# huangnengCSU/NanoSNP

Measured on NVIDIA B200. Metric: candidate sites/sec (s1+s2), higher is better.
Workload: dtype int32 counts, fp64 AF gate, fp16 hi/lo split x3 tensor-core model (fp32 accumulate)

## Files before the change

### nanosnp_b200/csrc/model_tc.cu

```cuda
#include <cuda_fp16.h>
#include <stdlib.h>
#include "model_common.cuh"
#include "tc_ptx.cuh"

namespace nsnp {
namespace {

constexpr int kRows = 128;
constexpr float kLog2e = 1.4426950408889634f;

__device__ __forceinline__ uint4 scale_hi(const uint4& hi) {
    const __half2 k = __float2half2_rn(1.0f / kTcLoScale);
    auto m = [&](uint32_t x) { __half2 t = *reinterpret_cast<__half2*>(&x); return h2_bits(__hmul2(t, k)); };
    return make_uint4(m(hi.x), m(hi.y), m(hi.z), m(hi.w));
}

template <int LAYER> struct TcCfg;
template <> struct TcCfg<0> { static constexpr int K = kTcK0, IN = kTcIn0, STEPS = 33; };
template <> struct TcCfg<1> { static constexpr int K = kTcK1, IN = kTcIn1, STEPS = 17; };

template <int LAYER, int CG> struct TcSmem {
    static constexpr int K = TcCfg<LAYER>::K;
    static constexpr int RB = 256 / CG;
    static constexpr size_t b_bytes = (size_t)K * RB * 2;
// ... 204 lines not shown
        }

        uint32_t vb[2][16];
        const uint32_t tacc = tmem_base + acc_cols + ((uint32_t)(quad * 32) << 16) + (uint32_t)(sub * UB) * 32u;
        tmem_ld16_nowait(tacc, vb[0]);
        tmem_wait_ld();
        float hv[8];
#pragma unroll
        for (int hb = 0; hb < 2 * UB; ++hb) {
            const int jl = hb >> 1, uh = hb & 1, jb = sub * UB + jl;
            if (hb + 1 < 2 * UB) tmem_ld16_nowait(tacc + (hb + 1) * 16, vb[(hb + 1) & 1]);
#pragma unroll
            for (int u = 0; u < 4; ++u) {
                const uint32_t* v = vb[hb & 1];
                const float* bq = sBias + jb * 32 + uh * 16 + u;
                const float bi_ = LAYER == 1 ? bq[0] : 0.f, bf_ = LAYER == 1 ? bq[4] : 0.f, bg_ = LAYER == 1 ? bq[8] : 0.f, bo_ = LAYER == 1 ? bq[12] : 0.f;
                const float xi_ = fminf(__uint_as_float(v[u]) + bi_, 36.f), xf_ = fminf(__uint_as_float(v[4 + u]) + bf_, 36.f);
                const float xg_ = fminf(__uint_as_float(v[8 + u]) + bg_, 36.f), xo_ = __uint_as_float(v[12 + u]) + bo_;
                const float ei = ex2_approx(xi_), ef = ex2_approx(xf_), eg = ex2_approx(xg_), eo = ex2_approx(xo_);
                const float pi = 1.f + ei, pf = 1.f + ef, pg = 1.f + eg;
                const float pig = pi * pg;
                const float num = fmaf(c[jl][uh * 4 + u], pig, fmaf(eg, 2.f * kLog2e, -2.f * kLog2e) * pf);
                const float cn = num * rcp_approx(pf * pig);
                c[jl][uh * 4 + u] = cn;
                const float ec = ex2_approx(cn);
                hv[uh * 4 + u] = (1.f - ec) * rcp_approx((1.f + eo) * (1.f + ec));
            }
            if (hb + 1 < 2 * UB) tmem_wait_ld();
            if (uh == 1) {
                const HiLo8 s = split8(hv);
                reinterpret_cast<uint4*>(sAhi + (IN / 8 + jb) * LBO_A)[row] = s.hi;
                reinterpret_cast<uint4*>(sAlo + (IN / 8 + jb) * LBO_A)[row] = s.lo;
                if (live) {
                    if (LAYER == 0) {
                        __half* o = h0_out + ((((size_t)blockIdx.x * kT + t) * 2) * 16 + (dir * 8 + jb)) * (kRows * 8) + row * 8;
                        *reinterpret_cast<uint4*>(o) = s.hi;
                        *reinterpret_cast<uint4*>(o + 16 * kRows * 8) = s.lo;
                    } else if (step == C::STEPS - 1) {
                        float4* o = reinterpret_cast<float4*>(h16 + site * 128 + dir * kH + jb * 8);
                        o[0] = make_float4(hv[0], hv[1], hv[2], hv[3]); o[1] = make_float4(hv[4], hv[5], hv[6], hv[7]);
                    }
                }
            }
        }
        if (more) store_x();
    }

    tc_fence_before();
    if (CG == 2) cluster_sync_all(); else __syncthreads();
    if (warp == 0) tmem_dealloc<CG>(tmem_base, kTmemCols);
}


__device__ __forceinline__ void mbar_arrive(uint64_t* bar) {
    asm volatile("mbarrier.arrive.shared::cta.b64 _, [%0];" ::"r"(smem_u32(bar)) : "memory");
}

constexpr int kP2GroupThreads = 256, kP2Threads = 2 * kP2GroupThreads;
struct P2Smem {
    static constexpr size_t b_bytes = (size_t)kTcK0 * 128 * 2;
    static constexpr size_t a_bytes = (size_t)kTcK0 * kRows * 2;
    static constexpr size_t sc_bytes = (size_t)kTcIn0 * kRows * 2;
    static constexpr size_t a_stride = 2 * a_bytes + sc_bytes;
    static constexpr size_t off_bhi = 0, off_blo = b_bytes, off_a = 2 * b_bytes, off_bar = off_a + 2 * a_stride, total = off_bar + 128;
};

__global__ void __launch_bounds__(kP2Threads, 1)
lstm0_pair2_kernel(const unsigned char* __restrict__ blob, const int32_t* __restrict__ xi, const float* __restrict__ xf,
                   __half* __restrict__ h0_out, int64_t n, const int32_t* __restrict__ pos, int64_t pos_bias, int npass)
{
    using S = P2Smem;
    constexpr int K = kTcK0, IN = kTcIn0, KB = K / 16, RB = 128, UB = 4;
    constexpr uint32_t LBO_A = kRows * 16, LBO_B = RB * 16, SBO = 128;
    extern __shared__ __align__(1024) unsigned char smem[];
    const int grp = (int)threadIdx.x / kP2GroupThreads;
    const int tid = (int)threadIdx.x - grp * kP2GroupThreads, lane = tid & 31, warp = tid >> 5;
    unsigned char* sBhi = smem + S::off_bhi; unsigned char* sBlo = smem + S::off_blo;
    unsigned char* sAhi = smem + S::off_a + grp * S::a_stride; unsigned char* sAlo = sAhi + S::a_bytes; unsigned char* sAsc = sAlo + S::a_bytes;
    uint64_t* bars = reinterpret_cast<uint64_t*>(smem + S::off_bar);
    uint64_t* barH = bars + grp;
    uint64_t* barReady = bars + 2 + grp;
    uint64_t* barTurn = bars + 4;
    uint32_t* tmem_slot = reinterpret_cast<uint32_t*>(smem + S::off_bar + 64);

    const int quad = warp & 3, sub = warp >> 2;
    const int row = quad * 32 + lane;
    const uint32_t cta_rank = cluster_ctarank();
    const int cluster_id = (int)(blockIdx.x >> 1);
    const int dir = cluster_id & 1;
    const int quad_stride = (int)(gridDim.x >> 2);
    const int n_quads = (int)((n + 4 * kRows - 1) / (4 * kRows));
    const int q0 = cluster_id >> 1;
    const int my_quads = q0 < n_quads ? (n_quads - q0 + quad_stride - 1) / quad_stride : 0;
    const int total_g = my_quads * kT;
    auto tile_of = [&](int qi) -> int64_t { return (int64_t)(q0 + qi * quad_stride) * 4 + (int64_t)cta_rank * 2 + grp; };

    if (threadIdx.x == 0) {
        mbar_init(bars + 0, 1); mbar_init(bars + 1, 1); mbar_init(bars + 2, 16); mbar_init(bars + 3, 16);
        mbar_init(bars + 4, 1); mbar_init(bars + 5, 1);
        fence_mbar_init();
    }
    if (threadIdx.x < 32) tmem_alloc<2>(tmem_slot, 512);
    {
        const uint4* ghi = reinterpret_cast<const uint4*>(blob + tc_off(0, dir, 0));
        const uint4* glo = reinterpret_cast<const uint4*>(blob + tc_off(0, dir, 1));
        uint4* dhi = reinterpret_cast<uint4*>(sBhi); uint4* dlo = reinterpret_cast<uint4*>(sBlo);
        for (int i = (int)threadIdx.x; i < (K / 8) * RB; i += kP2Threads) {
            const int ch = i / RB, r = i - ch * RB;
            const int g = ch * 256 + (int)cta_rank * RB + r;
            dhi[i] = __ldg(ghi + g); dlo[i] = __ldg(glo + g);
        }
        uint4* a = reinterpret_cast<uint4*>(sAhi);
        for (int i = tid; i < (int)(S::a_stride / 16); i += kP2GroupThreads) a[i] = make_uint4(0, 0, 0, 0);
    }
    __syncthreads();

    float c[UB][8];
#pragma unroll
    for (int j = 0; j < UB; ++j)
#pragma unroll
        for (int u = 0; u < 8; ++u) c[j][u] = 0.f;

    int2 xraw[8];
    int64_t win0 = 0;
    auto load_x = [&](int gstep) {
        const int qi = gstep / kT, st = gstep - qi * kT;
        const int t = dir == 0 ? st : (kT - 1 - st);
        int64_t site = tile_of(qi) * kRows + row;
        if (site >= n) site = n - 1;
        if (pos && st == 0) win0 = (int64_t)__ldg(pos + site) - pos_bias;
        const int2* g = pos ? reinterpret_cast<const int2*>(xi + (win0 + t) * kF)
                            : reinterpret_cast<const int2*>(xi ? (const void*)(xi + (site * kT + t) * kF) : (const void*)(xf + (site * kT + t) * kF));
        if (sub == 0) {
#pragma unroll
            for (int j = 0; j < 8; ++j) xraw[j] = ldg_nc_volatile(g + j);
        } else {
            xraw[0] = ldg_nc_volatile(g + 8);
        }
    };
    auto xval = [&](int j) -> float {
        const int2 p = xraw[j >> 1];
        const int b = (j & 1) ? p.y : p.x;
        return xi ? (float)b : __int_as_float(b);
    };
    auto store_x = [&]() {
        if (sub == 0) {
#pragma unroll
            for (int ch = 0; ch < 2; ++ch) {
                float v[8];
#pragma unroll
                for (int j = 0; j < 8; ++j) v[j] = xval(ch * 8 + j);
                const HiLo8 sp = split8(v);
                reinterpret_cast<uint4*>(sAhi + ch * LBO_A)[row] = sp.hi;
                reinterpret_cast<uint4*>(sAlo + ch * LBO_A)[row] = sp.lo;
                reinterpret_cast<uint4*>(sAsc + ch * LBO_A)[row] = scale_hi(sp.hi);
            }
        } else {
            const float v[8] = {xval(0), xval(1), 1.0f, 0.f, 0.f, 0.f, 0.f, 0.f};
            const HiLo8 sp = split8(v);
            reinterpret_cast<uint4*>(sAhi + 2 * LBO_A)[row] = sp.hi;
            reinterpret_cast<uint4*>(sAlo + 2 * LBO_A)[row] = sp.lo;
            reinterpret_cast<uint4*>(sAsc + 2 * LBO_A)[row] = scale_hi(sp.hi);
        }
    };
    auto report_ready = [&]() {
        fence_async_smem();
        tc_fence_before();
        __syncwarp();
        if (lane == 0) mbar_arrive_remote_relaxed(barReady, 0);
    };
    if (total_g > 0) { load_x(0); store_x(); }
    tc_fence_before();
    cluster_sync_all();
    tc_fence_after();
    if (total_g > 0) report_ready();

    const uint32_t tmem_base = *tmem_slot + (uint32_t)grp * 256u;
    const uint32_t a_hi = smem_u32(sAhi), a_lo = smem_u32(sAlo), a_sc = smem_u32(sAsc), b_hi = smem_u32(sBhi), b_lo = smem_u32(sBlo);
    constexpr uint32_t idesc = make_idesc(256, 256);
    const bool issuer = cta_rank == 0 && tid == 0;
    uint32_t phaseH = 0, phaseR = 0, phaseT = 0;
    if (cta_rank == 0 && threadIdx.x == 0) mbar_arrive(barTurn + 0);

    int step = 0, qi = 0;
    for (int g = 0; g < total_g; ++g) {
        const int t = dir == 0 ? step : (kT - 1 - step);
        const bool more = g + 1 < total_g;
        const int64_t tile_idx = tile_of(qi);
        const bool live = tile_idx * kRows + row < n;
        if (step == 0) {
#pragma unroll
            for (int j = 0; j < UB; ++j)
#pragma unroll
                for (int u = 0; u < 8; ++u) c[j][u] = 0.f;
        }
        if (issuer) {
            mbar_wait_cluster(barReady, phaseR);
            mbar_wait(barTurn + grp, phaseT);
            tc_fence_after();
#pragma unroll 1
            for (int pass = 0; pass < npass; ++pass) {
#pragma unroll 1
                for (int kb = 0; kb < (step == 0 ? IN / 16 : KB); ++kb) {
                    uint32_t aa = pass == 2 ? a_lo : a_hi;
                    if (pass == 1 && kb < IN / 16) aa = a_sc;
                    const uint32_t bb = pass == 1 ? b_lo : b_hi;
                    umma_f16<2>(tmem_base, make_desc(aa + kb * 2 * LBO_A, LBO_A, SBO), make_desc(bb + kb * 2 * LBO_B, LBO_B, SBO), idesc,
                                (pass | kb) ? 1u : 0u);
                }
            }
            umma_commit<2>(barH);
            mbar_arrive(barTurn + (grp ^ 1));
        }
        phaseR ^= 1; phaseT ^= 1;
        if (more) load_x(g + 1);
        mbar_wait(barH, phaseH);
        phaseH ^= 1;
        tc_fence_after();

        uint32_t vb[2][16];
        const uint32_t tacc = tmem_base + ((uint32_t)(quad * 32) << 16) + (uint32_t)(sub * UB) * 32u;
        tmem_ld16_nowait(tacc, vb[0]);
        tmem_wait_ld();
        float hv[8];
#pragma unroll
        for (int hb = 0; hb < 2 * UB; ++hb) {
            const int jl = hb >> 1, uh = hb & 1, jb = sub * UB + jl;
            if (hb + 1 < 2 * UB) tmem_ld16_nowait(tacc + (hb + 1) * 16, vb[(hb + 1) & 1]);
#pragma unroll
            for (int u = 0; u < 4; ++u) {
                const uint32_t* v = vb[hb & 1];
                const float xi_ = fminf(__uint_as_float(v[u]), 36.f), xf_ = fminf(__uint_as_float(v[4 + u]), 36.f);
                const float xg_ = fminf(__uint_as_float(v[8 + u]), 36.f), xo_ = __uint_as_float(v[12 + u]);
                const float ei = ex2_approx(xi_), ef = ex2_approx(xf_), eg = ex2_approx(xg_), eo = ex2_approx(xo_);
                const float pi = 1.f + ei, pf = 1.f + ef, pg = 1.f + eg;
                const float pig = pi * pg;
                const float num = fmaf(c[jl][uh * 4 + u], pig, fmaf(eg, 2.f * kLog2e, -2.f * kLog2e) * pf);
                const float cn = num * rcp_approx(pf * pig);
                c[jl][uh * 4 + u] = cn;
                const float ec = ex2_approx(cn);
                hv[uh * 4 + u] = (1.f - ec) * rcp_approx((1.f + eo) * (1.f + ec));
            }
            if (hb + 1 < 2 * UB) tmem_wait_ld();
            if (uh == 1) {
                const HiLo8 sp = split8(hv);
                reinterpret_cast<uint4*>(sAhi + (IN / 8 + jb) * LBO_A)[row] = sp.hi;
                if (npass == 3) reinterpret_cast<uint4*>(sAlo + (IN / 8 + jb) * LBO_A)[row] = sp.lo;
                if (live) {
                    __half* o = h0_out + ((((size_t)tile_idx * kT + t) * 2) * 16 + (dir * 8 + jb)) * (kRows * 8) + row * 8;
                    *reinterpret_cast<uint4*>(o) = sp.hi;
                    if (npass == 3) *reinterpret_cast<uint4*>(o + 16 * kRows * 8) = sp.lo;
                }
            }
        }
        if (more) { store_x(); report_ready(); }
        if (++step == kT) { step = 0; ++qi; }
    }

    tc_fence_before();
    cluster_sync_all();
    if (threadIdx.x < 32) tmem_dealloc<2>(*tmem_slot, 512);
}

struct P2Smem1 {
    static constexpr size_t b_bytes = (size_t)kTcK1 * 128 * 2;
    static constexpr size_t a_bytes = (size_t)kTcK1 * kRows * 2;
    static constexpr size_t off_b = 0, off_a = b_bytes, off_bias = off_a + 2 * a_bytes, off_bar = off_bias + 256 * sizeof(float), total = off_bar + 128;
};

__global__ void __launch_bounds__(kP2Threads, 1)
lstm1_pair2_kernel(const unsigned char* __restrict__ blob, const __half* __restrict__ h0_in, float* __restrict__ h16, int64_t n)
{
    using S = P2Smem1;
    constexpr int K = kTcK1, IN = kTcIn1, KB = K / 16, XB = IN / 16, RB = 128, UB = 4, kS = TcCfg<1>::STEPS;
    constexpr uint32_t LBO_A = kRows * 16, LBO_B = RB * 16, SBO = 128;
    constexpr uint32_t kPartBytes = 16u * kRows * 16u;
    extern __shared__ __align__(1024) unsigned char smem[];
    const int grp = (int)threadIdx.x / kP2GroupThreads;
    const int tid = (int)threadIdx.x - grp * kP2GroupThreads, lane = tid & 31, warp = tid >> 5;
    unsigned char* sB = smem + S::off_b;
    unsigned char* sA = smem + S::off_a + grp * S::a_bytes;
    float* sBias = reinterpret_cast<float*>(smem + S::off_bias);
    uint64_t* bars = reinterpret_cast<uint64_t*>(smem + S::off_bar);
    uint64_t* barH = bars + grp;
    uint64_t* barReady = bars + 2 + grp;
    uint64_t* barTurn = bars + 4;
    uint64_t* barIn = bars + 6 + grp;
    uint32_t* tmem_slot = reinterpret_cast<uint32_t*>(smem + S::off_bar + 64);

    const int quad = warp & 3, sub = warp >> 2;
    const int row = quad * 32 + lane;
    const uint32_t cta_rank = cluster_ctarank();
    const int cluster_id = (int)(blockIdx.x >> 1);
    const int dir = cluster_id & 1;
    const int quad_stride = (int)(gridDim.x >> 2);
    const int n_quads = (int)((n + 4 * kRows - 1) / (4 * kRows));
    const int64_t last_tile = (n + kRows - 1) / kRows - 1;
    const int q0 = cluster_id >> 1;
    const int my_quads = q0 < n_quads ? (n_quads - q0 + quad_stride - 1) / quad_stride : 0;
    const int total_g = my_quads * kS;
    auto tile_of = [&](int qi) -> int64_t { return (int64_t)(q0 + qi * quad_stride) * 4 + (int64_t)cta_rank * 2 + grp; };

    if (threadIdx.x == 0) {
        mbar_init(bars + 0, 1); mbar_init(bars + 1, 1); mbar_init(bars + 2, 16); mbar_init(bars + 3, 16);
        mbar_init(bars + 4, 1); mbar_init(bars + 5, 1); mbar_init(bars + 6, 1); mbar_init(bars + 7, 1);
        fence_mbar_init();
    }
    if (threadIdx.x < 32) tmem_alloc<2>(tmem_slot, 512);
    {
        const uint4* ghi = reinterpret_cast<const uint4*>(blob + tc_off(1, dir, 0));
        uint4* dhi = reinterpret_cast<uint4*>(sB);
        for (int i = (int)threadIdx.x; i < (K / 8) * RB; i += kP2Threads) {
            const int ch = i / RB, r = i - ch * RB;
            dhi[i] = __ldg(ghi + ch * 256 + (int)cta_rank * RB + r);
        }
        const float* gb = reinterpret_cast<const float*>(blob + kOffTcBias1) + dir * 256;
        for (int i = (int)threadIdx.x; i < 256; i += kP2Threads) sBias[i] = __ldg(gb + i);
    }
    __syncthreads();

    float c[UB][8];
#pragma unroll
    for (int j = 0; j < UB; ++j)
#pragma unroll
        for (int u = 0; u < 8; ++u) c[j][u] = 0.f;

    auto stage_in = [&](int gstep) {
        const int qi = gstep / kS, st = gstep - qi * kS;
        const int t = dir == 0 ? st : (kT - 1 - st);
        const int64_t tile = min(tile_of(qi), last_tile);
        mbar_expect_tx(barIn, kPartBytes);
        bulk_g2s(sA, h0_in + ((size_t)tile * kT + t) * (size_t)kPartBytes, kPartBytes, barIn);
    };
    auto report_ready = [&]() {
        fence_async_smem();
        tc_fence_before();
        __syncwarp();
        if (lane == 0) mbar_arrive_remote_relaxed(barReady, 0);
// ... 8 lines not shown
        report_ready();
    }

    const uint32_t tmem_base = *tmem_slot + (uint32_t)grp * 256u;
    const uint32_t a_hi = smem_u32(sA), b_hi = smem_u32(sB);
    constexpr uint32_t idesc = make_idesc(256, 256);
    const bool issuer = cta_rank == 0 && tid == 0;
    uint32_t phaseH = 0, phaseR = 0, phaseT = 0;
    if (cta_rank == 0 && threadIdx.x == 0) mbar_arrive(barTurn + 0);

    int step = 0, qi = 0;
    for (int g = 0; g < total_g; ++g) {
        const bool more = g + 1 < total_g;
        const int64_t site = tile_of(qi) * kRows + row;
        const bool live = site < n;
        if (step == 0) {
#pragma unroll
            for (int j = 0; j < UB; ++j)
#pragma unroll
                for (int u = 0; u < 8; ++u) c[j][u] = 0.f;
        }
        if (issuer) {
            mbar_wait_cluster(barReady, phaseR);
            mbar_wait(barTurn + grp, phaseT);
            tc_fence_after();
#pragma unroll 1
            for (int kb = 0; kb < (step == 0 ? XB : KB); ++kb)
                umma_f16<2>(tmem_base, make_desc(a_hi + kb * 2 * LBO_A, LBO_A, SBO), make_desc(b_hi + kb * 2 * LBO_B, LBO_B, SBO), idesc, kb ? 1u : 0u);
            umma_commit<2>(barH);
            mbar_arrive(barTurn + (grp ^ 1));
        }
        phaseR ^= 1; phaseT ^= 1;
        mbar_wait(barH, phaseH);
        phaseH ^= 1;
        tc_fence_after();
        if (more && tid == 0) stage_in(g + 1);

        uint32_t vb[2][16];
        const uint32_t tacc = tmem_base + ((uint32_t)(quad * 32) << 16) + (uint32_t)(sub * UB) * 32u;
        tmem_ld16_nowait(tacc, vb[0]);
        tmem_wait_ld();
        float hv[8];
#pragma unroll
        for (int hb = 0; hb < 2 * UB; ++hb) {
            const int jl = hb >> 1, uh = hb & 1, jb = sub * UB + jl;
            if (hb + 1 < 2 * UB) tmem_ld16_nowait(tacc + (hb + 1) * 16, vb[(hb + 1) & 1]);
#pragma unroll
            for (int u = 0; u < 4; ++u) {
                const uint32_t* v = vb[hb & 1];
                const float* bq = sBias + jb * 32 + uh * 16 + u;
                const float xi_ = fminf(__uint_as_float(v[u]) + bq[0], 36.f), xf_ = fminf(__uint_as_float(v[4 + u]) + bq[4], 36.f);
                const float xg_ = fminf(__uint_as_float(v[8 + u]) + bq[8], 36.f), xo_ = __uint_as_float(v[12 + u]) + bq[12];
                const float ei = ex2_approx(xi_), ef = ex2_approx(xf_), eg = ex2_approx(xg_), eo = ex2_approx(xo_);
                const float pi = 1.f + ei, pf = 1.f + ef, pg = 1.f + eg;
                const float pig = pi * pg;
                const float num = fmaf(c[jl][uh * 4 + u], pig, fmaf(eg, 2.f * kLog2e, -2.f * kLog2e) * pf);
                const float cn = num * rcp_approx(pf * pig);
                c[jl][uh * 4 + u] = cn;
                const float ec = ex2_approx(cn);
                hv[uh * 4 + u] = (1.f - ec) * rcp_approx((1.f + eo) * (1.f + ec));
            }
            if (hb + 1 < 2 * UB) tmem_wait_ld();
            if (uh == 1) {
                const HiLo8 sp = split8(hv);
                reinterpret_cast<uint4*>(sA + (IN / 8 + jb) * LBO_A)[row] = sp.hi;
                if (live && step == kS - 1) {
                    float4* o = reinterpret_cast<float4*>(h16 + site * 128 + dir * kH + jb * 8);
                    o[0] = make_float4(hv[0], hv[1], hv[2], hv[3]); o[1] = make_float4(hv[4], hv[5], hv[6], hv[7]);
                }
            }
        }
        if (more) {
            if (warp == 0) { mbar_wait(barIn, phaseIn); phaseIn ^= 1; }
            report_ready();
        }
        if (++step == kS) { step = 0; ++qi; }
    }

    tc_fence_before();
    cluster_sync_all();
    if (threadIdx.x < 32) tmem_dealloc<2>(*tmem_slot, 512);
}

template <class Kern, class... Args>
int launch_pair2(Kern kern, const char* name, size_t smem_bytes, int64_t m, cudaStream_t stream, Args... args) {
    const unsigned quads = (unsigned)((m + 4 * kRows - 1) / (4 * kRows));
    unsigned clusters = 2 * quads; if (clusters > (unsigned)kNumSMs / 2) clusters = ((unsigned)kNumSMs / 2) & ~1u;
    cudaLaunchConfig_t cfg = {};
    cfg.gridDim = dim3(2 * clusters, 1, 1);
    cfg.blockDim = dim3(kP2Threads, 1, 1);
    cfg.dynamicSmemBytes = smem_bytes;
    cfg.stream = stream;
    cudaLaunchAttribute attr[1];
    attr[0].id = cudaLaunchAttributeClusterDimension;
    attr[0].val.clusterDim.x = 2; attr[0].val.clusterDim.y = 1; attr[0].val.clusterDim.z = 1;
    cfg.attrs = attr; cfg.numAttrs = 1;
    const cudaError_t e = cudaLaunchKernelEx(&cfg, kern, args...);
    if (e != cudaSuccess) return set_error(NSNP_E_CUDA, "%s: %s", name, cudaGetErrorString(e));
    return NSNP_OK;
}

int launch_l0_pair2(const void* blob, const int32_t* xi, const float* xf, void* h0_out, int64_t m, const int32_t* pos, int64_t pos_bias, int npass, cudaStream_t stream) {
    static bool attr_done = false;
    if (!attr_done) {
        if (cudaFuncSetAttribute(lstm0_pair2_kernel, cudaFuncAttributeMaxDynamicSharedMemorySize, (int)P2Smem::total) != cudaSuccess)
            return cuda_status("cudaFuncSetAttribute(lstm0_pair2_kernel)");
        attr_done = true;
    }
    return launch_pair2(lstm0_pair2_kernel, "lstm0_pair2_kernel", P2Smem::total, m, stream, (const unsigned char*)blob, xi, xf, (__half*)h0_out, m, pos, pos_bias, npass);
}

int launch_l1_pair2(const void* blob, const void* h0_in, float* h16, int64_t m, cudaStream_t stream) {
    static bool attr_done = false;
    if (!attr_done) {
        if (cudaFuncSetAttribute(lstm1_pair2_kernel, cudaFuncAttributeMaxDynamicSharedMemorySize, (int)P2Smem1::total) != cudaSuccess)
            return cuda_status("cudaFuncSetAttribute(lstm1_pair2_kernel)");
        attr_done = true;
    }
    return launch_pair2(lstm1_pair2_kernel, "lstm1_pair2_kernel", P2Smem1::total, m, stream, (const unsigned char*)blob, (const __half*)h0_in, h16, m);
}

constexpr int kTtEpiWarps = 8, kTtLoadWarps = 4;
constexpr int kTtThreads = (kTtEpiWarps + kTtLoadWarps + 1) * 32;
struct TailSmem {
    static constexpr size_t w_bytes = kTcBytesTail;
    static constexpr size_t a_bytes = (size_t)128 * kRows * 2;
    static constexpr size_t off_whi = 0, off_wlo = w_bytes, off_ahi = 2 * w_bytes, off_alo = off_ahi + a_bytes,
                            off_head = off_alo + a_bytes,
                            off_bias = off_head + 256 * 24 * 4,
                            off_xch = off_bias + (256 + 32) * 4,
                            off_bar = off_xch + 128 * 12 * 4, total = off_bar + 64;
};

__device__ __forceinline__ void named_bar_sync(int id, int nthreads) { asm volatile("bar.sync %0, %1;" ::"r"(id), "r"(nthreads) : "memory"); }

__global__ void __launch_bounds__(kTtThreads, 1)
tail_tc_kernel(const unsigned char* __restrict__ blob, const float* __restrict__ h16, int64_t n_max, const int32_t* __restrict__ n_dev,
               float* __restrict__ gt, float* __restrict__ zy)
{
    using S = TailSmem;
    constexpr uint32_t LBO_A = kRows * 16, LBO_B = 256 * 16, SBO = 128;
    extern __shared__ __align__(1024) unsigned char smem[];
    unsigned char* sWhi = smem + S::off_whi; unsigned char* sWlo = smem + S::off_wlo;
    unsigned char* sAhi = smem + S::off_ahi; unsigned char* sAlo = smem + S::off_alo;
    float* sHead = reinterpret_cast<float*>(smem + S::off_head);
    float* sBias = reinterpret_cast<float*>(smem + S::off_bias);
    float* sXch = reinterpret_cast<float*>(smem + S::off_xch);
    uint64_t* bar = reinterpret_cast<uint64_t*>(smem + S::off_bar);
    uint32_t* tmem_slot = reinterpret_cast<uint32_t*>(smem + S::off_bar + 48);
    uint64_t* barH = bar; uint64_t* barIn = bar + 2; uint64_t* barFree = bar + 3;

    const int tid = threadIdx.x, lane = tid & 31, warp = tid >> 5;
    int64_t n = n_max;
    if (n_dev) { const int64_t nd = *n_dev; if (nd < n) n = nd; }
    const int n_tiles = (int)((n + kRows - 1) / kRows);
    const int my_tiles = (int)blockIdx.x < n_tiles ? (n_tiles - (int)blockIdx.x + (int)gridDim.x - 1) / (int)gridDim.x : 0;

    if (tid == 0) {
        mbar_init(barH, 1); mbar_init(barH + 1, 1); mbar_init(barIn, kTtLoadWarps);
        mbar_init(barFree, kTtEpiWarps); mbar_init(barFree + 1, kTtEpiWarps);
        fence_mbar_init();
    }
    if (warp == 0) tmem_alloc<1>(tmem_slot, 512);
    {
        const uint4* ghi = reinterpret_cast<const uint4*>(blob + kOffTcTail);
        const uint4* glo = reinterpret_cast<const uint4*>(blob + kOffTcTail + kTcBytesTail);
        uint4* dhi = reinterpret_cast<uint4*>(sWhi); uint4* dlo = reinterpret_cast<uint4*>(sWlo);
        for (int i = tid; i < (int)(S::w_bytes / 16); i += kTtThreads) { dhi[i] = __ldg(ghi + i); dlo[i] = __ldg(glo + i); }
        const float* fb = reinterpret_cast<const float*>(blob);
        for (int i = tid; i < 256 * 24; i += kTtThreads) sHead[i] = __ldg(fb + kOffHeadW + i);
        for (int i = tid; i < 256; i += kTtThreads) sBias[i] = __ldg(fb + kOffDenseB + i);
        if (tid < 24) sBias[256 + tid] = __ldg(fb + kOffHeadB + tid);
    }
    fence_async_smem();
    tc_fence_before();
    __syncthreads();
    tc_fence_after();
    const uint32_t tmem_base = *tmem_slot;

    if (warp == kTtEpiWarps + kTtLoadWarps) {
        if (lane == 0) {
            const uint32_t a_hi = smem_u32(sAhi), a_lo = smem_u32(sAlo), b_hi = smem_u32(sWhi), b_lo = smem_u32(sWlo);
            constexpr uint32_t idesc = make_idesc(128, 256);
            for (int g = 0; g < my_tiles; ++g) {
                const int b = g & 1;
                mbar_wait(barIn, (uint32_t)(g & 1));
                if (g >= 2) mbar_wait(barFree + b, (uint32_t)(((g >> 1) - 1) & 1));
                tc_fence_after();
                const uint32_t acc = tmem_base + (uint32_t)b * 256u;
#pragma unroll 1
                for (int kb = 0; kb < 8; ++kb) {
                    const uint64_t bh = make_desc(b_hi + kb * 2 * LBO_B, LBO_B, SBO), bl = make_desc(b_lo + kb * 2 * LBO_B, LBO_B, SBO);
                    const uint64_t ah = make_desc(a_hi + kb * 2 * LBO_A, LBO_A, SBO), al = make_desc(a_lo + kb * 2 * LBO_A, LBO_A, SBO);
                    umma_f16<1>(acc, ah, bh, idesc, kb == 0 ? 0u : 1u);
                    umma_f16<1>(acc, ah, bl, idesc, 1u);
                    umma_f16<1>(acc, al, bh, idesc, 1u);
                }
                umma_commit<1>(barH + b);
            }
        }
    } else if (warp >= kTtEpiWarps) {
        const int row = (warp - kTtEpiWarps) * 32 + lane;
// ... 75 lines not shown
                if (half == 0) {
#pragma unroll
                    for (int q = 0; q < 3; ++q) { const float4 v = x[q]; lg[12 * r + 4 * q] += v.x; lg[12 * r + 4 * q + 1] += v.y; lg[12 * r + 4 * q + 2] += v.z; lg[12 * r + 4 * q + 3] += v.w; }
                }
                named_bar_sync(1 + quad, 64);
            }
            if (half == 0 && site < n) {
                float m = lg[0];
#pragma unroll
                for (int j = 1; j < 21; ++j) m = fmaxf(m, lg[j]);
                float sum = 0.f;
#pragma unroll
                for (int j = 0; j < 21; ++j) { lg[j] = expf(lg[j] - m); sum += lg[j]; }
#pragma unroll
                for (int j = 0; j < 21; ++j) gt[site * 21 + j] = lg[j] / sum;
                const float m2 = fmaxf(lg[21], fmaxf(lg[22], lg[23]));
                const float e0 = expf(lg[21] - m2), e1 = expf(lg[22] - m2), e2 = expf(lg[23] - m2);
                const float s2 = e0 + e1 + e2;
                zy[site * 3 + 0] = e0 / s2; zy[site * 3 + 1] = e1 / s2; zy[site * 3 + 2] = e2 / s2;
            }
        }
    }

    tc_fence_before();
    __syncthreads();
    if (warp == 0) tmem_dealloc<1>(tmem_base, 512);
}

template <int LAYER, int CG, int NWQ, bool DEBUG>
int launch_one(const void* blob, const int32_t* xi, const float* xf, const void* h0_in, void* h0_out, float* h16, float* dbg,
               int64_t m, int dir_override, cudaStream_t stream)
{
    using S = TcSmem<LAYER, CG>;
    auto kern = lstm_tc_kernel<LAYER, CG, NWQ, DEBUG>;
    static bool attr_done = false;
    if (!attr_done) {
        if (cudaFuncSetAttribute(kern, cudaFuncAttributeMaxDynamicSharedMemorySize, (int)S::total) != cudaSuccess) return cuda_status("cudaFuncSetAttribute(lstm_tc_kernel)");
        attr_done = true;
    }
    unsigned gx = (unsigned)((m + kRows - 1) / kRows);
    if (CG == 2 && (gx & 1)) ++gx;
    cudaLaunchConfig_t cfg = {};
    cfg.gridDim = dim3(gx, DEBUG ? 1 : 2, 1);
    cfg.blockDim = dim3(128 * NWQ + (LAYER == 1 ? 32 : 0), 1, 1);
    cfg.dynamicSmemBytes = S::total;
    cfg.stream = stream;
    cudaLaunchAttribute attr[1];
    attr[0].id = cudaLaunchAttributeClusterDimension;
    attr[0].val.clusterDim.x = CG; attr[0].val.clusterDim.y = 1; attr[0].val.clusterDim.z = 1;
    cfg.attrs = attr; cfg.numAttrs = 1;
    const cudaError_t e = cudaLaunchKernelEx(&cfg, kern, (const unsigned char*)blob, xi, xf, (const __half*)h0_in, (__half*)h0_out, h16, dbg, m, dir_override);
    if (e != cudaSuccess) return set_error(NSNP_E_CUDA, "lstm_tc_kernel<%d,%d,%d>: %s", LAYER, CG, NWQ, cudaGetErrorString(e));
    return NSNP_OK;
}

}

int launch_tail_tc(const void* blob, const float* h16, int64_t n_max, const int32_t* n_dev, float* gt, float* zy, cudaStream_t stream) {
    using S = TailSmem;
    static bool attr_done = false;
    if (!attr_done) {
        if (cudaFuncSetAttribute(tail_tc_kernel, cudaFuncAttributeMaxDynamicSharedMemorySize, (int)S::total) != cudaSuccess)
            return cuda_status("cudaFuncSetAttribute(tail_tc_kernel)");
        attr_done = true;
    }
    const int64_t n_tiles = (n_max + kRows - 1) / kRows;
    const int grid = (int)(n_tiles < kNumSMs ? n_tiles : kNumSMs);
    tail_tc_kernel<<<grid, kTtThreads, S::total, stream>>>((const unsigned char*)blob, h16, n_max, n_dev, gt, zy);
    return cuda_status("tail_tc_kernel");
}

int launch_lstm_tc(const void* blob, const int32_t* xi, const float* xf, void* h0, float* h16, int64_t m, const int32_t* pos, int64_t pos_bias, int npass, cudaStream_t stream) {
    {
        ProfScope prof(NSNP_PROF_LSTM0, stream);
        static const int variant = [] { const char* v = getenv("NSNP_L0_VARIANT"); return v ? atoi(v) : 1; }();
        if (pos && variant != 1) return set_error(NSNP_E_UNSUPPORTED, "window reads from the count tensor need the default layer-0 kernel");
        if (int e = variant == 1 ? launch_l0_pair2(blob, xi, xf, h0, m, pos, pos_bias, npass, stream)
                                 : launch_one<0, 2, 2, false>(blob, xi, xf, nullptr, h0, nullptr, nullptr, m, npass << 16, stream)) return e;
    }
    ProfScope prof(NSNP_PROF_LSTM1, stream);
    static const int pf = [] { const char* v = getenv("NSNP_L1_PREFETCH"); return v ? atoi(v) : 1; }();
    static const int l1_variant = [] { const char* v = getenv("NSNP_L1_VARIANT"); return v ? atoi(v) : 1; }();
    if (npass == 1 && l1_variant == 1) return launch_l1_pair2(blob, h0, h16, m, stream);
    return launch_one<1, 2, 4, false>(blob, nullptr, nullptr, h0, nullptr, h16, nullptr, m, (pf << 8) | (npass << 16), stream);
}

int debug_tc_gates(const void* blob, const int32_t* xi, int layer, int dir, int cg, const void* h0, float* gates_out, int64_t m, cudaStream_t stream) {
    if (layer == 0 && cg == 1) return launch_one<0, 1, 2, true>(blob, xi, nullptr, nullptr, nullptr, nullptr, gates_out, m, dir, stream);
    if (layer == 0 && cg == 2) return launch_one<0, 2, 2, true>(blob, xi, nullptr, nullptr, nullptr, nullptr, gates_out, m, dir, stream);
    if (layer == 1 && cg == 2) return launch_one<1, 2, 4, true>(blob, nullptr, nullptr, h0, nullptr, nullptr, gates_out, m, dir, stream);
    return set_error(NSNP_E_UNSUPPORTED, "debug_tc_gates: layer %d with cta_group %d is not built", layer, cg);
}

int pack_tc_weights(const nsnp_model_weights_t* w, unsigned char* blob) {
    for (int layer = 0; layer < 2; ++layer) {
        const int K = layer == 0 ? kTcK0 : kTcK1, IN = layer == 0 ? kTcIn0 : kTcIn1, nin = layer == 0 ? kF : 128;
        for (int d = 0; d < 2; ++d) {
            __half* hi = reinterpret_cast<__half*>(blob + tc_off(layer, d, 0));
            __half* lo = reinterpret_cast<__half*>(blob + tc_off(layer, d, 1));
            const float *wih = w->w_ih[layer][d], *whh = w->w_hh[layer][d], *bi = w->b_ih[layer][d], *bh = w->b_hh[layer][d];
            for (int n = 0; n < 256; ++n) {
                const int jb = n >> 5, uh = (n >> 4) & 1, gate = (n >> 2) & 3, u4 = n & 3;
                const int rowi = gate * kH + jb * 8 + uh * 4 + u4;
                for (int k = 0; k < K; ++k) {
                    float v = 0.f;
                    if (k < nin) v = wih[rowi * nin + k];
                    else if (layer == 0 && k == nin) v = bi[rowi] + bh[rowi];
                    else if (k >= IN) v = whh[rowi * kH + (k - IN)];
                    v *= gate == 2 ? -2.0f * kLog2e : -kLog2e;
                    const float scale = (layer == 0 && k < IN) ? kTcLoScale : 1.0f;
                    const __half h = __float2half_rn(v);
                    const __half l = __float2half_rn((v - __half2float(h)) * scale);
                    const size_t idx = ((size_t)(k >> 3) * 256 + n) * 8 + (k & 7);
                    hi[idx] = h; lo[idx] = l;
                }
                if (layer == 1) reinterpret_cast<float*>(blob + kOffTcBias1)[d * 256 + n] = (bi[rowi] + bh[rowi]) * (gate == 2 ? -2.0f * kLog2e : -kLog2e);
            }
        }
    }
    {
        const float* Wd = reinterpret_cast<const float*>(blob) + kOffDenseW;
        __half* hi = reinterpret_cast<__half*>(blob + kOffTcTail);
        __half* lo = reinterpret_cast<__half*>(blob + kOffTcTail + kTcBytesTail);
        for (int n = 0; n < 256; ++n)
            for (int k = 0; k < 128; ++k) {
                const float v = Wd[(size_t)k * 256 + n];
                const __half h = __float2half_rn(v);
                const size_t idx = ((size_t)(k >> 3) * 256 + n) * 8 + (k & 7);
                hi[idx] = h; lo[idx] = __float2half_rn(v - __half2float(h));
            }
    }
    return NSNP_OK;
}

}

extern "C" int nsnp_debug_lstm_tc_gates(const void* blob_dev, const int32_t* x_i32_dev, int layer, int dir, int cg, const void* h0_dev,
                                        float* gates_out_dev, int64_t m, void* stream)
{
    if (!blob_dev || !gates_out_dev || m <= 0 || dir < 0 || dir > 1) return nsnp::set_error(NSNP_E_INVALID, "nsnp_debug_lstm_tc_gates: bad argument");
    if (nsnp_device_count() == 0) return nsnp::set_error(NSNP_E_NO_DEVICE, "no CUDA device (there is no CPU fallback)");
    return nsnp::debug_tc_gates(blob_dev, x_i32_dev, layer, dir, cg, h0_dev, gates_out_dev, m, (cudaStream_t)stream);
}
```

### nanosnp_b200/csrc/tc_ptx.cuh

```cuda
#pragma once
#include <cuda_fp16.h>
#include <stdint.h>

namespace nsnp {
namespace {

__device__ __forceinline__ uint32_t smem_u32(const void* p) { return (uint32_t)__cvta_generic_to_shared(p); }
__device__ __forceinline__ void mbar_init(uint64_t* bar, uint32_t count) {
    asm volatile("mbarrier.init.shared::cta.b64 [%0], %1;" ::"r"(smem_u32(bar)), "r"(count) : "memory");
}
__device__ __forceinline__ void fence_mbar_init() { asm volatile("fence.mbarrier_init.release.cluster;" ::: "memory"); }
__device__ __forceinline__ void mbar_wait(uint64_t* bar, uint32_t parity) {
    asm volatile(
        "{\n\t.reg .pred P1;\n\t"
        "WAIT_LOOP:\n\t"
        "mbarrier.try_wait.parity.shared::cta.b64 P1, [%0], %1;\n\t"
        "@P1 bra DONE;\n\t"
        "bra WAIT_LOOP;\n\t"
        "DONE:\n\t}"
        ::"r"(smem_u32(bar)), "r"(parity) : "memory");
}
__device__ __forceinline__ void mbar_wait_cluster(uint64_t* bar, uint32_t parity) {
    asm volatile(
        "{\n\t.reg .pred P1;\n\t"
        "WAIT_LOOP_C:\n\t"
        "mbarrier.try_wait.parity.acquire.cluster.shared::cta.b64 P1, [%0], %1;\n\t"
        "@P1 bra DONE_C;\n\t"
        "bra WAIT_LOOP_C;\n\t"
        "DONE_C:\n\t}"
        ::"r"(smem_u32(bar)), "r"(parity) : "memory");
}
__device__ __forceinline__ void mbar_arrive_remote_relaxed(uint64_t* bar, uint32_t target_cta) {
    uint32_t raddr;
    asm volatile("mapa.shared::cluster.u32 %0, %1, %2;" : "=r"(raddr) : "r"(smem_u32(bar)), "r"(target_cta));
    asm volatile("mbarrier.arrive.relaxed.cluster.shared::cluster.b64 _, [%0];" ::"r"(raddr) : "memory");
}
__device__ __forceinline__ void fence_async_smem() { asm volatile("fence.proxy.async.shared::cta;" ::: "memory"); }
__device__ __forceinline__ void tc_fence_before() { asm volatile("tcgen05.fence::before_thread_sync;" ::: "memory"); }
__device__ __forceinline__ void tc_fence_after() { asm volatile("tcgen05.fence::after_thread_sync;" ::: "memory"); }
__device__ __forceinline__ void cluster_sync_all() {
    asm volatile("barrier.cluster.arrive.release.aligned;\n\tbarrier.cluster.wait.acquire.aligned;" ::: "memory");
}
__device__ __forceinline__ void cluster_sync_exec() {
    asm volatile("barrier.cluster.arrive.relaxed.aligned;\n\tbarrier.cluster.wait.aligned;" ::: "memory");
}
__device__ __forceinline__ uint32_t cluster_ctarank() { uint32_t r; asm volatile("mov.u32 %0, %%cluster_ctarank;" : "=r"(r)); return r; }

template <int CG> __device__ __forceinline__ void tmem_alloc(uint32_t* dst_smem, uint32_t ncols) {
    if (CG == 1) {
        asm volatile("tcgen05.alloc.cta_group::1.sync.aligned.shared::cta.b32 [%0], %1;" ::"r"(smem_u32(dst_smem)), "r"(ncols) : "memory");
        asm volatile("tcgen05.relinquish_alloc_permit.cta_group::1.sync.aligned;" ::: "memory");
    } else {
        asm volatile("tcgen05.alloc.cta_group::2.sync.aligned.shared::cta.b32 [%0], %1;" ::"r"(smem_u32(dst_smem)), "r"(ncols) : "memory");
        asm volatile("tcgen05.relinquish_alloc_permit.cta_group::2.sync.aligned;" ::: "memory");
    }
}
template <int CG> __device__ __forceinline__ void tmem_dealloc(uint32_t taddr, uint32_t ncols) {
    if (CG == 1) asm volatile("tcgen05.dealloc.cta_group::1.sync.aligned.b32 %0, %1;" ::"r"(taddr), "r"(ncols) : "memory");
    else asm volatile("tcgen05.dealloc.cta_group::2.sync.aligned.b32 %0, %1;" ::"r"(taddr), "r"(ncols) : "memory");
}
template <int CG> __device__ __forceinline__ void umma_f16(uint32_t tmem_d, uint64_t adesc, uint64_t bdesc, uint32_t idesc, uint32_t accumulate) {
    if (CG == 1)
        asm volatile("{\n\t.reg .pred p;\n\tsetp.ne.b32 p, %4, 0;\n\ttcgen05.mma.cta_group::1.kind::f16 [%0], %1, %2, %3, p;\n\t}"
                     ::"r"(tmem_d), "l"(adesc), "l"(bdesc), "r"(idesc), "r"(accumulate) : "memory");
    else
        asm volatile("{\n\t.reg .pred p;\n\tsetp.ne.b32 p, %4, 0;\n\ttcgen05.mma.cta_group::2.kind::f16 [%0], %1, %2, %3, p;\n\t}"
                     ::"r"(tmem_d), "l"(adesc), "l"(bdesc), "r"(idesc), "r"(accumulate) : "memory");
}
__device__ __forceinline__ void umma_tf32(uint32_t tmem_d, uint64_t adesc, uint64_t bdesc, uint32_t idesc, uint32_t accumulate) {
    asm volatile("{\n\t.reg .pred p;\n\tsetp.ne.b32 p, %4, 0;\n\ttcgen05.mma.cta_group::1.kind::tf32 [%0], %1, %2, %3, p;\n\t}"
                 ::"r"(tmem_d), "l"(adesc), "l"(bdesc), "r"(idesc), "r"(accumulate) : "memory");
}
template <int CG> __device__ __forceinline__ void umma_commit(uint64_t* bar) {
    if (CG == 1)
        asm volatile("tcgen05.commit.cta_group::1.mbarrier::arrive::one.shared::cluster.b64 [%0];" ::"r"(smem_u32(bar)) : "memory");
    else
        asm volatile("tcgen05.commit.cta_group::2.mbarrier::arrive::one.shared::cluster.multicast::cluster.b64 [%0], %1;"
                     ::"r"(smem_u32(bar)), "h"((uint16_t)3) : "memory");
}
__device__ __forceinline__ void tmem_ld32(uint32_t taddr, float (&v)[32]) {
    uint32_t r[32];
    asm volatile(
        "tcgen05.ld.sync.aligned.32x32b.x32.b32 "
        "{%0, %1, %2, %3, %4, %5, %6, %7, %8, %9, %10, %11, %12, %13, %14, %15, "
        "%16, %17, %18, %19, %20, %21, %22, %23, %24, %25, %26, %27, %28, %29, %30, %31}, [%32];\n\t"
        "tcgen05.wait::ld.sync.aligned;"
        : "=r"(r[0]), "=r"(r[1]), "=r"(r[2]), "=r"(r[3]), "=r"(r[4]), "=r"(r[5]), "=r"(r[6]), "=r"(r[7]),
          "=r"(r[8]), "=r"(r[9]), "=r"(r[10]), "=r"(r[11]), "=r"(r[12]), "=r"(r[13]), "=r"(r[14]), "=r"(r[15]),
          "=r"(r[16]), "=r"(r[17]), "=r"(r[18]), "=r"(r[19]), "=r"(r[20]), "=r"(r[21]), "=r"(r[22]), "=r"(r[23]),
          "=r"(r[24]), "=r"(r[25]), "=r"(r[26]), "=r"(r[27]), "=r"(r[28]), "=r"(r[29]), "=r"(r[30]), "=r"(r[31])
        : "r"(taddr) : "memory");
#pragma unroll
    for (int i = 0; i < 32; ++i) v[i] = __uint_as_float(r[i]);
}
__device__ __forceinline__ void tmem_ld16_nowait(uint32_t taddr, uint32_t (&r)[16]) {
    asm volatile(
        "tcgen05.ld.sync.aligned.32x32b.x16.b32 "
        "{%0, %1, %2, %3, %4, %5, %6, %7, %8, %9, %10, %11, %12, %13, %14, %15}, [%16];"
        : "=r"(r[0]), "=r"(r[1]), "=r"(r[2]), "=r"(r[3]), "=r"(r[4]), "=r"(r[5]), "=r"(r[6]), "=r"(r[7]),
          "=r"(r[8]), "=r"(r[9]), "=r"(r[10]), "=r"(r[11]), "=r"(r[12]), "=r"(r[13]), "=r"(r[14]), "=r"(r[15])
        : "r"(taddr) : "memory");
}
__device__ __forceinline__ void tmem_wait_ld() { asm volatile("tcgen05.wait::ld.sync.aligned;" ::: "memory"); }
__device__ __forceinline__ int2 ldg_nc_volatile(const int2* p) {
    int2 v;
    asm volatile("ld.global.nc.v2.s32 {%0, %1}, [%2];" : "=r"(v.x), "=r"(v.y) : "l"(p) : "memory");
    return v;
}
__device__ __forceinline__ float ex2_approx(float x) { float y; asm("ex2.approx.ftz.f32 %0, %1;" : "=f"(y) : "f"(x)); return y; }
__device__ __forceinline__ float rcp_approx(float x) { float y; asm("rcp.approx.ftz.f32 %0, %1;" : "=f"(y) : "f"(x)); return y; }

__device__ __forceinline__ uint64_t make_desc(uint32_t saddr, uint32_t lbo_bytes, uint32_t sbo_bytes) {
    return (uint64_t)((saddr >> 4) & 0x3FFF) | ((uint64_t)((lbo_bytes >> 4) & 0x3FFF) << 16) |
           ((uint64_t)((sbo_bytes >> 4) & 0x3FFF) << 32) | (1ull << 46);
}
__host__ __device__ constexpr uint32_t make_idesc(int m, int n) { return (1u << 4) | ((uint32_t)(n >> 3) << 17) | ((uint32_t)(m >> 4) << 24); }

struct HiLo8 { uint4 hi, lo; };
// ... 29 lines not shown
```

Baseline: 41.67 million.

## Skip lo-part input MMAs when the x tile has no fp16 residual

```diff
diff --git a/nanosnp_b200/csrc/model_tc.cu b/nanosnp_b200/csrc/model_tc.cu
--- a/nanosnp_b200/csrc/model_tc.cu
+++ b/nanosnp_b200/csrc/model_tc.cu
@@ -310,6 +310,8 @@
     uint64_t* barReady = bars + 2 + grp;
     uint64_t* barTurn = bars + 4;
     uint32_t* tmem_slot = reinterpret_cast<uint32_t*>(smem + S::off_bar + 64);
+    uint32_t* xlo_words = reinterpret_cast<uint32_t*>(smem + S::off_bar + 72);
+    uint32_t* xlo_word = xlo_words + grp;
 
     const int quad = warp & 3, sub = warp >> 2;
     const int row = quad * 32 + lane;
@@ -326,6 +328,7 @@
     if (threadIdx.x == 0) {
         mbar_init(bars + 0, 1); mbar_init(bars + 1, 1); mbar_init(bars + 2, 16); mbar_init(bars + 3, 16);
         mbar_init(bars + 4, 1); mbar_init(bars + 5, 1);
+        xlo_words[0] = 0; xlo_words[1] = 0;
         fence_mbar_init();
     }
     if (threadIdx.x < 32) tmem_alloc<2>(tmem_slot, 512);
@@ -371,7 +374,8 @@
         const int b = (j & 1) ? p.y : p.x;
         return xi ? (float)b : __int_as_float(b);
     };
-    auto store_x = [&]() {
+    auto store_x = [&]() -> bool {
+        uint32_t lo = 0;
         if (sub == 0) {
 #pragma unroll
             for (int ch = 0; ch < 2; ++ch) {
@@ -382,6 +386,7 @@
                 reinterpret_cast<uint4*>(sAhi + ch * LBO_A)[row] = sp.hi;
                 reinterpret_cast<uint4*>(sAlo + ch * LBO_A)[row] = sp.lo;
                 reinterpret_cast<uint4*>(sAsc + ch * LBO_A)[row] = scale_hi(sp.hi);
+                lo |= sp.lo.x | sp.lo.y | sp.lo.z | sp.lo.w;
             }
         } else {
             const float v[8] = {xval(0), xval(1), 1.0f, 0.f, 0.f, 0.f, 0.f, 0.f};
@@ -389,19 +394,26 @@
             reinterpret_cast<uint4*>(sAhi + 2 * LBO_A)[row] = sp.hi;
             reinterpret_cast<uint4*>(sAlo + 2 * LBO_A)[row] = sp.lo;
             reinterpret_cast<uint4*>(sAsc + 2 * LBO_A)[row] = scale_hi(sp.hi);
-        }
+            lo = sp.lo.x | sp.lo.y | sp.lo.z | sp.lo.w;
+        }
+        return lo != 0;
     };
-    auto report_ready = [&]() {
+    auto report_ready = [&](bool xlo) {
         fence_async_smem();
         tc_fence_before();
         __syncwarp();
-        if (lane == 0) mbar_arrive_remote_relaxed(barReady, 0);
+        const bool any = __any_sync(~0u, xlo);
+        if (lane == 0) {
+            if (any) { red_or_remote(xlo_word, 1u, 0); mbar_arrive_remote_release(barReady, 0); }
+            else mbar_arrive_remote_relaxed(barReady, 0);
+        }
     };
-    if (total_g > 0) { load_x(0); store_x(); }
+    bool xlo = false;
+    if (total_g > 0) { load_x(0); xlo = store_x(); }
     tc_fence_before();
     cluster_sync_all();
     tc_fence_after();
-    if (total_g > 0) report_ready();
+    if (total_g > 0) report_ready(xlo);
 
     const uint32_t tmem_base = *tmem_slot + (uint32_t)grp * 256u;
     const uint32_t a_hi = smem_u32(sAhi), a_lo = smem_u32(sAlo), a_sc = smem_u32(sAsc), b_hi = smem_u32(sBhi), b_lo = smem_u32(sBlo);
@@ -422,14 +434,17 @@
 #pragma unroll
                 for (int u = 0; u < 8; ++u) c[j][u] = 0.f;
         }
+        if (more) load_x(g + 1);
         if (issuer) {
             mbar_wait_cluster(barReady, phaseR);
             mbar_wait(barTurn + grp, phaseT);
             tc_fence_after();
+            const bool xlo_step = atomicExch(xlo_word, 0u) != 0u;
 #pragma unroll 1
             for (int pass = 0; pass < npass; ++pass) {
 #pragma unroll 1
                 for (int kb = 0; kb < (step == 0 ? IN / 16 : KB); ++kb) {
+                    if (pass == 2 && kb < IN / 16 && !xlo_step) continue;
                     uint32_t aa = pass == 2 ? a_lo : a_hi;
                     if (pass == 1 && kb < IN / 16) aa = a_sc;
                     const uint32_t bb = pass == 1 ? b_lo : b_hi;
@@ -441,10 +456,10 @@
             mbar_arrive(barTurn + (grp ^ 1));
         }
         phaseR ^= 1; phaseT ^= 1;
-        if (more) load_x(g + 1);
         mbar_wait(barH, phaseH);
         phaseH ^= 1;
         tc_fence_after();
+        if (more) xlo = store_x();
 
         uint32_t vb[2][16];
         const uint32_t tacc = tmem_base + ((uint32_t)(quad * 32) << 16) + (uint32_t)(sub * UB) * 32u;
@@ -481,7 +496,7 @@
                 }
             }
         }
-        if (more) { store_x(); report_ready(); }
+        if (more) report_ready(xlo);
         if (++step == kT) { step = 0; ++qi; }
     }
 
diff --git a/nanosnp_b200/csrc/tc_ptx.cuh b/nanosnp_b200/csrc/tc_ptx.cuh
--- a/nanosnp_b200/csrc/tc_ptx.cuh
+++ b/nanosnp_b200/csrc/tc_ptx.cuh
@@ -34,6 +34,16 @@
     uint32_t raddr;
     asm volatile("mapa.shared::cluster.u32 %0, %1, %2;" : "=r"(raddr) : "r"(smem_u32(bar)), "r"(target_cta));
     asm volatile("mbarrier.arrive.relaxed.cluster.shared::cluster.b64 _, [%0];" ::"r"(raddr) : "memory");
+}
+__device__ __forceinline__ void mbar_arrive_remote_release(uint64_t* bar, uint32_t target_cta) {
+    uint32_t raddr;
+    asm volatile("mapa.shared::cluster.u32 %0, %1, %2;" : "=r"(raddr) : "r"(smem_u32(bar)), "r"(target_cta));
+    asm volatile("mbarrier.arrive.release.cluster.shared::cluster.b64 _, [%0];" ::"r"(raddr) : "memory");
+}
+__device__ __forceinline__ void red_or_remote(uint32_t* word, uint32_t v, uint32_t target_cta) {
+    uint32_t raddr;
+    asm volatile("mapa.shared::cluster.u32 %0, %1, %2;" : "=r"(raddr) : "r"(smem_u32(word)), "r"(target_cta));
+    asm volatile("red.relaxed.cluster.shared::cluster.or.b32 [%0], %1;" ::"r"(raddr), "r"(v) : "memory");
 }
 __device__ __forceinline__ void fence_async_smem() { asm volatile("fence.proxy.async.shared::cta;" ::: "memory"); }
 __device__ __forceinline__ void tc_fence_before() { asm volatile("tcgen05.fence::before_thread_sync;" ::: "memory"); }
```

Result: no change. 41.98 million (median of 6 runs) (+0.7%).

## Add persistent cluster-pair layer-1 LSTM kernel with double-buffered TMEM accumulators

Applied to the files above, without the earlier changes.

```diff
diff --git a/nanosnp_b200/csrc/model_tc.cu b/nanosnp_b200/csrc/model_tc.cu
--- a/nanosnp_b200/csrc/model_tc.cu
+++ b/nanosnp_b200/csrc/model_tc.cu
@@ -656,13 +656,189 @@
     if (threadIdx.x < 32) tmem_dealloc<2>(*tmem_slot, 512);
 }
 
+constexpr int kL1Threads = 128 * 4 + 32;
+
+__global__ void __launch_bounds__(kL1Threads, 1)
+lstm1_persist_kernel(const unsigned char* __restrict__ blob, const __half* __restrict__ h0_in, float* __restrict__ h16, int64_t n,
+                     int npass, int l2_prefetch)
+{
+    using S = TcSmem<1, 2>;
+    constexpr int IN = kTcIn1, KB = kTcK1 / 16, XB = IN / 16, RB = S::RB, NWQ = 4, UB = 8 / NWQ, kS = TcCfg<1>::STEPS;
+    constexpr int kEpiWarps = 4 * NWQ;
+    constexpr uint32_t LBO_A = kRows * 16, LBO_B = RB * 16, SBO = 128;
+    constexpr uint32_t kPartBytes = 16u * kRows * 16u;
+    extern __shared__ __align__(1024) unsigned char smem[];
+    unsigned char* sBhi = smem + S::off_bhi; unsigned char* sBlo = smem + S::off_blo;
+    unsigned char* sAhi = smem + S::off_ahi; unsigned char* sAlo = smem + S::off_alo;
+    float* sBias = reinterpret_cast<float*>(smem + S::off_bias);
+    uint64_t* bar = reinterpret_cast<uint64_t*>(smem + S::off_bar);
+    uint64_t* barH = bar;
+    uint64_t* barX = bar + 1;
+    uint64_t* barS = bar + 2;
+    uint32_t* tmem_slot = reinterpret_cast<uint32_t*>(smem + S::off_bar + 32);
+
+    const int tid = threadIdx.x, lane = tid & 31, warp = tid >> 5;
+    const bool producer = warp == kEpiWarps;
+    const int quad = warp & 3, sub = producer ? 0 : (warp >> 2);
+    const int row = quad * 32 + lane;
+    const uint32_t cta_rank = cluster_ctarank();
+    const int cluster_id = (int)(blockIdx.x >> 1);
+    const int dir = cluster_id & 1;
+    const int pair_stride = (int)(gridDim.x >> 2);
+    const int64_t last_tile = (n + kRows - 1) / kRows - 1;
+    const int n_pairs = (int)((n + 2 * kRows - 1) / (2 * kRows));
+    const int p0 = cluster_id >> 1;
+    const int my_pairs = p0 < n_pairs ? (n_pairs - p0 + pair_stride - 1) / pair_stride : 0;
+    const int total_g = my_pairs * kS;
+    auto tile_of = [&](int pi) -> int64_t { return (int64_t)(p0 + pi * pair_stride) * 2 + cta_rank; };
+
+    if (tid == 0) { mbar_init(barH, 1); mbar_init(barX, 1); mbar_init(barS, 1); fence_mbar_init(); }
+    if (warp == 0) tmem_alloc<2>(tmem_slot, 512);
+    {
+        const uint4* ghi = reinterpret_cast<const uint4*>(blob + tc_off(1, dir, 0));
+        const uint4* glo = reinterpret_cast<const uint4*>(blob + tc_off(1, dir, 1));
+        uint4* dhi = reinterpret_cast<uint4*>(sBhi); uint4* dlo = reinterpret_cast<uint4*>(sBlo);
+        for (int i = tid; i < (kTcK1 / 8) * RB; i += kL1Threads) {
+            const int ch = i / RB, r = i - ch * RB;
+            const int g = ch * 256 + (int)cta_rank * RB + r;
+            dhi[i] = __ldg(ghi + g); dlo[i] = __ldg(glo + g);
+        }
+        const float* gb = reinterpret_cast<const float*>(blob + kOffTcBias1) + dir * 256;
+        for (int i = tid; i < 256; i += kL1Threads) sBias[i] = __ldg(gb + i);
+    }
+    __syncthreads();
+
+    auto rows_of = [&](int g) -> const __half* {
+        const int st = g % kS, t = dir == 0 ? st : (kT - 1 - st);
+        return h0_in + ((size_t)min(tile_of(g / kS), last_tile) * kT + t) * kPartBytes;
+    };
+    auto stage = [&](int g) {
+        const __half* src = rows_of(g);
+        mbar_expect_tx(barS, 2 * kPartBytes);
+        bulk_g2s(sAhi, src, kPartBytes, barS);
+        bulk_g2s(sAlo, src + kPartBytes / 2, kPartBytes, barS);
+        if (l2_prefetch && g + 1 < total_g) bulk_prefetch_l2(rows_of(g + 1), 2 * kPartBytes);
+    };
+
+    tc_fence_before();
+    cluster_sync_all();
+    tc_fence_after();
+    uint32_t phaseH = 0, phaseX = 0, phaseS = 0;
+    if (total_g > 0) {
+        if (producer && lane == 0) stage(0);
+        mbar_wait(barS, phaseS); phaseS ^= 1;
+        tc_fence_before();
+        cluster_sync_all();
+        tc_fence_after();
+    }
+    const uint32_t tmem_base = *tmem_slot;
+    const uint32_t a_hi = smem_u32(sAhi), a_lo = smem_u32(sAlo), b_hi = smem_u32(sBhi), b_lo = smem_u32(sBlo);
+    constexpr uint32_t idesc = make_idesc(256, 256);
+    const bool issuer = cta_rank == 0 && tid == 0;
+    auto issue = [&](int kb0, int kb1, uint32_t tmem_d, uint32_t acc) {
+#pragma unroll 1
+        for (int pass = 0; pass < npass; ++pass) {
+#pragma unroll 1
+            for (int kb = kb0; kb < kb1; ++kb) {
+                const uint32_t aa = pass == 2 ? a_lo : a_hi, bb = pass == 1 ? b_lo : b_hi;
+                umma_f16<2>(tmem_d, make_desc(aa + kb * 2 * LBO_A, LBO_A, SBO), make_desc(bb + kb * 2 * LBO_B, LBO_B, SBO), idesc, acc);
+                acc = 1;
+            }
+        }
+    };
+    if (total_g > 0) {
+        if (issuer) { tc_fence_after(); issue(0, XB, tmem_base, 0); umma_commit<2>(barX); }
+        if (producer) {
+            mbar_wait(barX, phaseX); phaseX ^= 1;
+            if (lane == 0 && total_g > 1) stage(1);
+        }
+    }
+
+    float c[UB][8];
+    int step = 0, pi = 0;
+    for (int g = 0; g < total_g; ++g) {
+        const bool more = g + 1 < total_g;
+        const uint32_t acc_cols = (uint32_t)(g & 1) * 256u;
+        if (more) { mbar_wait(barS, phaseS); phaseS ^= 1; }
+        fence_async_smem();
+        tc_fence_before();
+        cluster_sync_exec();
+        if (issuer) {
+            tc_fence_after();
+            if (step > 0) issue(XB, KB, tmem_base + acc_cols, 1);
+            umma_commit<2>(barH);
+            if (more) { issue(0, XB, tmem_base + (acc_cols ^ 256u), 0); umma_commit<2>(barX); }
+        }
+        if (producer) {
+            if (more) {
+                mbar_wait(barX, phaseX); phaseX ^= 1;
+                if (lane == 0 && g + 2 < total_g) stage(g + 2);
+            }
+        } else {
+            const int64_t site = tile_of(pi) * kRows + row;
+            const bool live = site < n;
+            if (step == 0) {
+#pragma unroll
+                for (int j = 0; j < UB; ++j)
+#pragma unroll
+                    for (int u = 0; u < 8; ++u) c[j][u] = 0.f;
+            }
+            mbar_wait(barH, phaseH);
+            phaseH ^= 1;
+            tc_fence_after();
+
+            uint32_t vb[2][16];
+            const uint32_t tacc = tmem_base + acc_cols + ((uint32_t)(quad * 32) << 16) + (uint32_t)(sub * UB) * 32u;
+            tmem_ld16_nowait(tacc, vb[0]);
+            tmem_wait_ld();
+            float hv[8];
+#pragma unroll
+            for (int hb = 0; hb < 2 * UB; ++hb) {
+                const int jl = hb >> 1, uh = hb & 1, jb = sub * UB + jl;
+                if (hb + 1 < 2 * UB) tmem_ld16_nowait(tacc + (hb + 1) * 16, vb[(hb + 1) & 1]);
+#pragma unroll
+                for (int u = 0; u < 4; ++u) {
+                    const uint32_t* v = vb[hb & 1];
+                    const float* bq = sBias + jb * 32 + uh * 16 + u;
+                    const float xi_ = fminf(__uint_as_float(v[u]) + bq[0], 36.f), xf_ = fminf(__uint_as_float(v[4 + u]) + bq[4], 36.f);
+                    const float xg_ = fminf(__uint_as_float(v[8 + u]) + bq[8], 36.f), xo_ = __uint_as_float(v[12 + u]) + bq[12];
+                    const float ei = ex2_approx(xi_), ef = ex2_approx(xf_), eg = ex2_approx(xg_), eo = ex2_approx(xo_);
+                    const float pi_ = 1.f + ei, pf = 1.f + ef, pg = 1.f + eg;
+                    const float pig = pi_ * pg;
+                    const float num = fmaf(c[jl][uh * 4 + u], pig, fmaf(eg, 2.f * kLog2e, -2.f * kLog2e) * pf);
+                    const float cn = num * rcp_approx(pf * pig);
+                    c[jl][uh * 4 + u] = cn;
+                    const float ec = ex2_approx(cn);
+                    hv[uh * 4 + u] = (1.f - ec) * rcp_approx((1.f + eo) * (1.f + ec));
+                }
+                if (hb + 1 < 2 * UB) tmem_wait_ld();
+                if (uh == 1) {
+                    const HiLo8 s = split8(hv);
+                    reinterpret_cast<uint4*>(sAhi + (IN / 8 + jb) * LBO_A)[row] = s.hi;
+                    reinterpret_cast<uint4*>(sAlo + (IN / 8 + jb) * LBO_A)[row] = s.lo;
+                    if (live && step == kS - 1) {
+                        float4* o = reinterpret_cast<float4*>(h16 + site * 128 + dir * kH + jb * 8);
+                        o[0] = make_float4(hv[0], hv[1], hv[2], hv[3]); o[1] = make_float4(hv[4], hv[5], hv[6], hv[7]);
+                    }
+                }
+            }
+        }
+        if (++step == kS) { step = 0; ++pi; }
+    }
+
+    tc_fence_before();
+    cluster_sync_all();
+    if (warp == 0) tmem_dealloc<2>(tmem_base, 512);
+}
+
 template <class Kern, class... Args>
-int launch_pair2(Kern kern, const char* name, size_t smem_bytes, int64_t m, cudaStream_t stream, Args... args) {
-    const unsigned quads = (unsigned)((m + 4 * kRows - 1) / (4 * kRows));
-    unsigned clusters = 2 * quads; if (clusters > (unsigned)kNumSMs / 2) clusters = ((unsigned)kNumSMs / 2) & ~1u;
+int launch_persistent(Kern kern, const char* name, size_t smem_bytes, int threads, int cluster_tiles, int64_t m, cudaStream_t stream,
+                      Args... args) {
+    const unsigned units = (unsigned)((m + cluster_tiles * kRows - 1) / (cluster_tiles * kRows));
+    unsigned clusters = 2 * units; if (clusters > (unsigned)kNumSMs / 2) clusters = ((unsigned)kNumSMs / 2) & ~1u;
     cudaLaunchConfig_t cfg = {};
     cfg.gridDim = dim3(2 * clusters, 1, 1);
-    cfg.blockDim = dim3(kP2Threads, 1, 1);
+    cfg.blockDim = dim3(threads, 1, 1);
     cfg.dynamicSmemBytes = smem_bytes;
     cfg.stream = stream;
     cudaLaunchAttribute attr[1];
@@ -681,7 +857,8 @@
             return cuda_status("cudaFuncSetAttribute(lstm0_pair2_kernel)");
         attr_done = true;
     }
-    return launch_pair2(lstm0_pair2_kernel, "lstm0_pair2_kernel", P2Smem::total, m, stream, (const unsigned char*)blob, xi, xf, (__half*)h0_out, m, pos, pos_bias, npass);
+    return launch_persistent(lstm0_pair2_kernel, "lstm0_pair2_kernel", P2Smem::total, kP2Threads, 4, m, stream, (const unsigned char*)blob, xi, xf,
+                             (__half*)h0_out, m, pos, pos_bias, npass);
 }
 
 int launch_l1_pair2(const void* blob, const void* h0_in, float* h16, int64_t m, cudaStream_t stream) {
@@ -691,7 +868,20 @@
             return cuda_status("cudaFuncSetAttribute(lstm1_pair2_kernel)");
         attr_done = true;
     }
-    return launch_pair2(lstm1_pair2_kernel, "lstm1_pair2_kernel", P2Smem1::total, m, stream, (const unsigned char*)blob, (const __half*)h0_in, h16, m);
+    return launch_persistent(lstm1_pair2_kernel, "lstm1_pair2_kernel", P2Smem1::total, kP2Threads, 4, m, stream, (const unsigned char*)blob,
+                             (const __half*)h0_in, h16, m);
+}
+
+int launch_l1_persist(const void* blob, const void* h0_in, float* h16, int64_t m, int npass, int l2_prefetch, cudaStream_t stream) {
+    using S = TcSmem<1, 2>;
+    static bool attr_done = false;
+    if (!attr_done) {
+        if (cudaFuncSetAttribute(lstm1_persist_kernel, cudaFuncAttributeMaxDynamicSharedMemorySize, (int)S::total) != cudaSuccess)
+            return cuda_status("cudaFuncSetAttribute(lstm1_persist_kernel)");
+        attr_done = true;
+    }
+    return launch_persistent(lstm1_persist_kernel, "lstm1_persist_kernel", S::total, kL1Threads, 2, m, stream, (const unsigned char*)blob,
+                             (const __half*)h0_in, h16, m, npass, l2_prefetch);
 }
 
 constexpr int kTtEpiWarps = 8, kTtLoadWarps = 4;
@@ -933,6 +1123,8 @@
     static const int pf = [] { const char* v = getenv("NSNP_L1_PREFETCH"); return v ? atoi(v) : 1; }();
     static const int l1_variant = [] { const char* v = getenv("NSNP_L1_VARIANT"); return v ? atoi(v) : 1; }();
     if (npass == 1 && l1_variant == 1) return launch_l1_pair2(blob, h0, h16, m, stream);
+    static const int persist = [] { const char* v = getenv("NSNP_L1_PERSIST"); return v ? atoi(v) : 1; }();
+    if (persist) return launch_l1_persist(blob, h0, h16, m, npass, pf, stream);
     return launch_one<1, 2, 4, false>(blob, nullptr, nullptr, h0, nullptr, h16, nullptr, m, (pf << 8) | (npass << 16), stream);
 }
 
```

Measured after the change: 41.21 million before, 42.23 million after, median of 6. +2.5%, better.
